# VITA-Group/mm-hand

Hardware: AMD Instinct MI355X
Metric: 256x256 hand images/sec (G+D step) (higher is better)
Workload: dtype f32; 1 GPU; RHD-shaped 256x256, per-GPU batch 32, fp32 (Winograd F(6x6,3x3) on the 3x3 stack), G(9 PATBlocks, ngf64)+D_PB+D_PP+L1/perceptual/GAN+Adam, --norm instance, dropout on; VGG19[:4] weights: random-init (seed 1234): NOT the reference's pretrained objective; global_batch=32, parallelism=dp1

## Files before the change

### include/mmhand_hip.h

```cpp
#ifndef MMHAND_HIP_H
#define MMHAND_HIP_H

#include <stddef.h>
#include <stdint.h>

#ifdef __cplusplus
extern "C" {
#endif
#pragma GCC visibility push(default)

typedef void* mmh_stream_t;

enum { MMH_PAD_ZERO = 0, MMH_PAD_REFLECT = 1 };
enum { MMH_ACT_NONE = 0, MMH_ACT_RELU = 1, MMH_ACT_TANH = 2 };
enum { MMH_F32 = 0, MMH_BF16 = 1, MMH_FP16 = 2 };

typedef struct mmh_conv_desc {
    int32_t B, H, W;
    int32_t Cin, Cout;
    int32_t kh, kw;
    int32_t stride;
    int32_t pad;
    int32_t pad_mode;
    int32_t Ho, Wo;
// ... 301 lines not shown
size_t mmh_conv7_head_dgrad_lp16_ws_bytes(const mmh_conv_desc* d);
int mmh_conv7_head_dgrad_lp16(const mmh_conv_desc* d, const void* dy, const void* w, void* dx, int dx_is16, void* ws,
                              size_t ws_bytes, const void* zeros, mmh_stream_t s);

int mmh_conv7_n4_lp16_supported(const mmh_conv_desc* d, int mode);
size_t mmh_conv7_n4_lp16_ws_bytes(const mmh_conv_desc* d, int mode);
int mmh_conv7_n4_lp16(const mmh_conv_desc* d, int mode, const void* x16, const void* w,
                      const void* bias, void* y, int act, void* ws, size_t ws_bytes,
                      const void* zeros, mmh_stream_t s);

int mmh_conv7_stem_wgrad_supported(const mmh_conv_desc* d);
size_t mmh_conv7_stem_wgrad_ws_bytes(const mmh_conv_desc* d);
int mmh_conv7_stem_wgrad(const mmh_conv_desc* d, const void* x, const void* dy, void* dw,
                         void* ws, size_t ws_bytes, int accumulate, mmh_stream_t s);

int mmh_adam_step(void* p, const void* g, void* m, void* v, int64_t n,
                  float lr, float beta1, float beta2, float eps, int step,
                  float grad_scale, const void* skip_flag, const void* loss_scale,
                  mmh_stream_t s);

int mmh_adam_step_dev(void* p, const void* g, void* m, void* v, int64_t n, const void* lr, float beta1, float beta2,
                      float eps, void* step, float grad_scale, const void* skip_flag, const void* loss_scale, void* coef,
                      mmh_stream_t s);

int mmh_set_dropout_salt(const void* salt_u64);
int mmh_u64_add(void* value_u64, uint64_t inc, mmh_stream_t s);

int mmh_pool_exchange(void* pool, const void* images, void* out, const void* src_idx, const void* dst_idx, int B,
                      int64_t elems_per_image, mmh_stream_t s);

// ... 110 lines not shown
```

### mmhand_amd/csrc/common.h

```cpp
#pragma once
#include <hip/hip_runtime.h>
#include <cstdarg>
#include <cstdio>
#include <cstdint>
#include "../../include/mmhand_hip.h"

namespace mmh {

char* err_buf();
int fail(const char* fmt, ...);

inline int check_launch(const char* what) {
    hipError_t e = hipGetLastError();
    if (e != hipSuccess) return fail("%s: %s", what, hipGetErrorString(e));
    return 0;
}

inline hipStream_t as_stream(mmh_stream_t s) { return reinterpret_cast<hipStream_t>(s); }

inline int64_t cdiv(int64_t a, int64_t b) { return (a + b - 1) / b; }

int wino6_weights(const float* w, float* U, int Cin, int Cout, int flip_transpose, hipStream_t st);
int wino6_weights_multi(const long long* table, int n, long long total_blocks, hipStream_t st);
int wino6_input(const float* x, float* V, int B, int H, int W, int C, int reflect, int xcd, hipStream_t st);
// ... 16 lines not shown
                       hipStream_t st);
bool dgrad_s2_halo_ok(const mmh_conv_desc* d, int dx_cs, int act);
int launch_dgrad_s2_halo(const mmh_conv_desc* d, const void* dy, const void* w, const void* bias, void* dx, int dx_cs,
                         int act, hipStream_t st);
extern int g_dgrad_s2_halo, g_dgrad_s2_dbg;
bool wgrad_s2_strip_ok(const mmh_conv_desc* d);
size_t wgrad_s2_strip_ws_bytes(const mmh_conv_desc* d);
int launch_wgrad_s2_strip(const mmh_conv_desc* d, const void* x, const void* dy, void* dw, void* ws, size_t ws_bytes,
                          int accumulate, hipStream_t st);
extern int g_wgrad_s2_strip;
bool stem_f32_ok(const mmh_conv_desc* d);
int stem_f32_stats_chunks(const mmh_conv_desc* d);
int launch_stem_f32(const mmh_conv_desc* d, const void* x, const void* w, const void* bias, void* y, int act, float* stats,
                    hipStream_t st);
extern int g_stem_f32, g_stem_f32_dbg, g_stem_f32_levels;
bool wino_wgrad_dma_ok(int64_t tiles, int Cin, int Cout, int nbatch);
size_t wino_wgrad_dma_ws_bytes(int64_t tiles, int Cin, int Cout, int nbatch);
int launch_wino_wgrad_dma(const float* V, const float* Yh, int64_t tiles, int Cin, int Cout, int nbatch, float* ws, float* dU,
                          hipStream_t st);
extern int g_wino_wgrad_dma;
int launch_slab_reduce(const float* slab, float* dw, int64_t n4_total, int splits, int accumulate, int64_t n4, hipStream_t st);
bool conv_s2f_ok(const mmh_conv_desc* d, int mode);
bool conv_s1f_ok(const mmh_conv_desc* d, int mode);
int conv_s2f_stats_chunks(const mmh_conv_desc* d);
int launch_conv_s2f(const mmh_conv_desc* d, const void* x16, const void* w16, const void* bias, void* y, int y_is16, int act,
                    const void* zeros, hipStream_t st, float* stats = nullptr, int mode = 0);
bool conv_s2d_ok(const mmh_conv_desc* d, int mode);
int launch_conv_s2d(const mmh_conv_desc* d, const void* g16, const void* w16, const void* bias, void* dx, int dx_is16, int act,
                    const void* zeros, hipStream_t st);
extern int g_lp16_s2f;
// ... 18 lines not shown
```

### mmhand_amd/csrc/conv_igemm.hip

```cpp
#include <algorithm>
#include <cstring>
#include "device_prims.h"

namespace {
using namespace mmh::dev;

typedef __bf16 bf16x4 __attribute__((ext_vector_type(4)));
typedef __bf16 bf16x2 __attribute__((ext_vector_type(2)));
typedef _Float16 f16x4 __attribute__((ext_vector_type(4)));
typedef _Float16 f16x2 __attribute__((ext_vector_type(2)));
__device__ __forceinline__ bf16x4 to_bf16x4(float4 v) {
    bf16x4 r;
    r[0] = (__bf16)v.x; r[1] = (__bf16)v.y; r[2] = (__bf16)v.z; r[3] = (__bf16)v.w;
    return r;
}
template <bool H16>
__device__ __forceinline__ bf16x4 to_lp4(float4 v) {
    if (H16) {
        f16x4 r;
        r[0] = (_Float16)v.x; r[1] = (_Float16)v.y; r[2] = (_Float16)v.z; r[3] = (_Float16)v.w;
        return __builtin_bit_cast(bf16x4, r);
    }
    return to_bf16x4(v);
}
// ... 2923 lines not shown
        {"wino_wgrad_dma", &mmh::g_wino_wgrad_dma},
        {"stem_f32_dbg", &mmh::g_stem_f32_dbg},
        {"slab_reduce_par", &mmh::g_slab_reduce_par},
        {"dgrad_s2_dbg", &mmh::g_dgrad_s2_dbg},
        {"lp16_dbg", &mmh::g_lp16_dbg},
        {"lp16_wgrad_ring", &mmh::g_lp16_wgrad_ring},
        {"lp16_wgrad_s2", &mmh::g_lp16_wgrad_s2},
        {"border_bn64", &g_border_bn64},
        {"wino_gemm_occ", &g_wino_gemm_occ},
        {"wino_gemm_levels", &g_wino_gemm_levels},
        {"wino_gemm_bn", &g_wino_gemm_bn},
        {"wino_bf16_occ", &g_wino_bf16_occ},
        {"wino_bf16_bk", &g_wino_bf16_bk},
        {"wino_wgrad_bn256", &g_wino_wgrad_bn256},
        {"wino_wgrad_slots", &g_wino_wgrad_slots},
    };
    *count = (int)(sizeof(table) / sizeof(table[0]));
    return table;
}
const OptionEntry* find_option(const char* key) {
    int n = 0;
    const OptionEntry* t = option_table(&n);
    for (int i = 0; i < n; ++i)
        if (!strcmp(key, t[i].name)) return &t[i];
    return nullptr;
}

}

extern "C" {
// ... 493 lines not shown
```

### mmhand_amd/lib.py

```python
import ctypes as C
import os

_HERE = os.path.dirname(os.path.abspath(__file__))
LIB_PATH = os.environ.get("MMH_LIB_PATH") or os.path.join(_HERE, "libmmhand_hip.so")

PAD_ZERO, PAD_REFLECT = 0, 1
ACT_NONE, ACT_RELU, ACT_TANH = 0, 1, 2
F32, BF16, FP16 = 0, 1, 2
U8 = 3


class ConvDesc(C.Structure):
    _fields_ = [(n, C.c_int32) for n in (
        "B", "H", "W", "Cin", "Cout", "kh", "kw", "stride", "pad", "pad_mode",
        "Ho", "Wo", "x_cs", "y_cs", "dtype")]


class PlaneSrc(C.Structure):
    _fields_ = [("ptr", C.c_void_p), ("C", C.c_int32),
                ("sb", C.c_int64), ("sc", C.c_int64), ("sh", C.c_int64), ("sw", C.c_int64)]


class ImageSrc(C.Structure):
    _fields_ = [("ptr", C.c_void_p), ("dtype", C.c_int32), ("scale", C.c_float), ("offset", C.c_float),
# ... 36 lines not shown
    "mmh_norm_stats_merge2": (_i, [_vp, _i, _i, _i, _vp, _sz, _vp, _vp, _vp]),
    "mmh_norm_stats_merge_finalize": (_i, [_vp, _i, _i, _i, _d, _f, _vp, _vp, _vp, _vp, _vp, _vp]),
    "mmh_wino_wgrad_gemm_ws_bytes": (_sz, [_i64, _i, _i, _i]),
    "mmh_wino_wgrad_gemm": (_i, [_vp, _vp, _i64, _i, _i, _i, _i, _vp, _sz, _vp, _vp]),
    "mmh_wino_dw": (_i, [_vp, _i, _i, _i, _vp, _i, _vp]),
    "mmh_conv2d_dgrad_border_ws_bytes": (_sz, [_DP]),
    "mmh_conv2d_dgrad_border": (_i, [_DP, _vp, _vp, _vp, _vp, _sz, _i, _i, _vp]),
    "mmh_conv7_thin_fprop": (_i, [_DP, _vp, _vp, _vp, _vp, _i, _vp]),
    "mmh_conv7_thin_dgrad_ws_bytes": (_sz, [_DP]),
    "mmh_conv7_thin_dgrad": (_i, [_DP, _vp, _vp, _vp, _vp, _sz, _i, _vp]),
    "mmh_conv7_thin_wgrad_ws_bytes": (_sz, [_DP]),
    "mmh_conv7_thin_wgrad": (_i, [_DP, _vp, _vp, _vp, _vp, _sz, _i, _vp]),
    "mmh_conv7_stem_wgrad_supported": (_i, [_DP]),
    "mmh_conv7_stem_wgrad_ws_bytes": (_sz, [_DP]),
    "mmh_conv7_stem_wgrad": (_i, [_DP, _vp, _vp, _vp, _vp, _sz, _i, _vp]),
    "mmh_conv2d_wgrad_ws_bytes": (_sz, [_DP]),
    "mmh_conv2d_wgrad": (_i, [_DP, _vp, _vp, _vp, _vp, _sz, _i, _i, _vp]),
    "mmh_convT2d_fprop": (_i, [_DP, _vp, _vp, _vp, _vp, _i, _i, _vp]),
    "mmh_convT2d_dgrad": (_i, [_DP, _vp, _vp, _vp, _vp]),
    "mmh_convT2d_wgrad": (_i, [_DP, _vp, _vp, _vp, _vp, _sz, _i, _i, _vp]),
    "mmh_reflect_fold": (_i, [_vp, _vp, _i, _i, _i, _i, _i, _vp]),
    "mmh_prep_weights_bf16": (_i, [_vp, _i, _i, _i, _vp, _vp, _vp]),
    "mmh_prep_weights_bf16_flat": (_i, [_vp, _i, _i, _i, _vp, _vp]),
    "mmh_prep_weights_fp16": (_i, [_vp, _i, _i, _i, _vp, _vp, _vp]),
    "mmh_prep_weights_fp16_flat": (_i, [_vp, _i, _i, _i, _vp, _vp]),
    "mmh_cvt_lp16": (_i, [_vp, _i64, _i, _vp, _vp]),
    "mmh_conv_lp16_supported": (_i, [_DP, _i]),
    "mmh_conv_lp16": (_i, [_DP, _i, _vp, _vp, _vp, _vp, _i, _i, _vp, _vp]),
    "mmh_conv_lp16_stats_chunks": (_i, [_DP]),
    "mmh_conv_lp16_fprop_stats": (_i, [_DP, _vp, _vp, _vp, _vp, _vp, _vp, _vp]),
# ... 163 lines not shown
```

### mmhand_amd/mmhand_model.py

```python
import os
import random
from collections import OrderedDict

import torch
import torch.distributed as dist

from . import lib as L
from . import ops
from .networks import Discriminator, Generator, VGGHead, discriminators_lockstep
from .ops import pad4
from .options import check_exact_fwd, check_resize_inputs


MERGE_D_PASSES = os.environ.get("MMH_MERGE_D", "1") != "0"
_LAST_BUCKET_LOG = None


def get_norm_layer(norm_type="instance"):
    if norm_type in ("batch", "instance"):
        return norm_type
    raise NotImplementedError("normalization layer [%s] is not found" % norm_type)


def get_scheduler(optimizer, opt):
# ... 257 lines not shown
        ops.set_dropout_seed((int(seed) * 0x9E3779B97F4A7C15 + 0x5EED0001 + rank * 0xD1B54A32D192ED03) % (1 << 64))
        norm = get_norm_layer(opt.norm)
        input_nc = [opt.H_input_nc, opt.P_input_nc * 2, opt.D_input_nc * 2]
        self.netG = Generator(input_nc, opt.output_nc, opt.ngf, norm, not opt.no_dropout,
                              n_blocks=getattr(opt, "G_n_blocks", 9),
                              n_downsampling=opt.G_n_downsampling)
        self.netG.to(self.device).init_weights(opt.init_type, seed)
        nets = [self.netG]
        if self.isTrain:
            self.netD_PB = Discriminator(opt.H_input_nc + opt.P_input_nc, opt.ndf, norm,
                                         not opt.no_dropout_D, opt.n_layers_D,
                                         n_downsampling=opt.D_n_downsampling)
            self.netD_PP = Discriminator(opt.H_input_nc + opt.H_input_nc, opt.ndf, norm,
                                         not opt.no_dropout_D, opt.n_layers_D,
                                         n_downsampling=opt.D_n_downsampling)
            self.netD_PB.to(self.device).init_weights(opt.init_type, seed + 1)
            self.netD_PP.to(self.device).init_weights(opt.init_type, seed + 2)
            nets += [self.netD_PB, self.netD_PP]
        if not self.isTrain or opt.continue_train:
            self.load_network()
        for n in nets:
            n.flatten_parameters()
        level = str(getattr(opt, "opt_level", "O0")).upper()
        if level not in ("O0", "O1", "O2", "O1_FP16", "O2_FP16", "BF16"):
            raise ValueError("--opt_level %r: expected O0 | O1 | O2 | O1_FP16 | O2_FP16 | BF16 (apex's O3 = "
                             "pure fp16 weights is 'not recommended' by the reference and not built)"
                             % (opt.opt_level,))
        self.bf16 = 2 if level.endswith("_FP16") else level in ("O1", "O2", "BF16")
        self.loss_scaling = self.isTrain and level != "O0" and level != "BF16"
        for n in nets:
# ... 592 lines not shown
```

### mmhand_amd/networks.py

```python
import functools
import math

import torch
import torch.nn as nn

from . import lib as L
from . import ops
from .ops import pad4


class ConvParam(nn.Module):

    def __init__(self, cin, cout, k, bias, transposed=False):
        super().__init__()
        self.cin, self.cout, self.k, self.transposed = cin, cout, k, transposed
        a, b = (pad4(cout), pad4(cin)) if transposed else (pad4(cin), pad4(cout))
        self.weight = nn.Parameter(torch.zeros(k, k, a, b))
        self.bias = nn.Parameter(torch.zeros(pad4(cout))) if bias else None

    def logical_weight(self):
        w = self.weight.detach()
        if self.transposed:
            return w.permute(3, 2, 0, 1)[: self.cin, : self.cout]
        return w.permute(3, 2, 0, 1)[: self.cout, : self.cin]

    def set_logical(self, weight=None, bias=None):
        with torch.no_grad():
            if weight is not None:
                self.weight.zero_()
                self.logical_weight().copy_(weight)
            if bias is not None and self.bias is not None:
                self.bias.zero_()
                self.bias[: self.cout].copy_(bias)
# ... 217 lines not shown
            elif isinstance(m, NormParam):
                with torch.no_grad():
                    m.weight.copy_(1.0 + torch.randn(m.weight.shape, generator=g) * 0.02)
                    m.bias.zero_()
        return self

    def conv(self, cp, x, stride=1, pad=0, reflect=False, act=L.ACT_NONE, dx_channels=0, y_lp=False, to_norm=False,
             g_defer=False, res_tok=None, x_twin=None):
        x16 = None
        if isinstance(x, tuple):
            x, x16 = x
        if isinstance(x16, ops.NormDefer):
            return ops.Conv2dFn.apply(x, cp.weight, cp.bias, stride, pad, reflect, act, self.bf16, dx_channels, None,
                                      False, bool(to_norm and self.norm == "instance" and self.training), x16, g_defer)
        nb = bool(to_norm and self.training and (self.norm == "instance" or cp.bias is None))
        if x16 is not None:
            res_tok = None
        if y_lp:
            p, y16 = ops.Conv2dFn.apply(x, cp.weight, cp.bias, stride, pad, reflect, act, self.bf16, dx_channels, x16, True, nb,
                                        None, False, res_tok, x_twin)
            return p, y16
        return ops.Conv2dFn.apply(x, cp.weight, cp.bias, stride, pad, reflect, act, self.bf16, dx_channels, x16, False, nb,
                                  None, g_defer, res_tok, x_twin)

    def _lp_edge(self, cp, stride=1, reflect=True):
        if not (self.bf16 and self.training and cp is not None and cp.k == 3):
            return 0
        ws = cp.weight.shape
        if cp.transposed:
            return self.bf16 if ops.convT_lp16_ok(ws[3], ws[2], self.bf16) else 0
# ... 156 lines not shown
    def __init__(self, input_nc, output_nc, ngf=64, norm_layer=nn.BatchNorm2d, use_dropout=False,
                 n_blocks=6, gpu_ids=[], padding_type="reflect", n_downsampling=2):
        assert type(input_nc) == list and len(input_nc) == 3, \
            "The AttModule take input_nc in format of list only!!"
        assert n_blocks >= 0
        if padding_type != "reflect":
            raise NotImplementedError("padding [%s] is not implemented" % padding_type)
        super().__init__(norm_layer, use_dropout)
        self.input_nc, self.output_nc, self.ngf = list(input_nc), output_nc, ngf
        self.n_blocks, self.n_down = n_blocks, n_downsampling
        self.gpu_ids = gpu_ids
        m = self.model = Bag()
        for s, nc in zip((1, 2, 3), input_nc):
            d = m.put(f"stream{s}_down", Bag())
            self._conv(d, 1, nc, ngf, 7)
            self._normp(d, 2, ngf)
            for i in range(n_downsampling):
                c = ngf * 2 ** i
                self._conv(d, 4 + 3 * i, c, 2 * c, 3)
                self._normp(d, 5 + 3 * i, 2 * c)
        dim = ngf * 2 ** n_downsampling
        att = m.put("att", Bag())
        i2 = 6 if use_dropout else 5
        for b in range(n_blocks):
            blk = att.put(b, Bag())
            for s in (1, 2, 3):
                cb = blk.put(f"conv_block_stream{s}", Bag())
                wide = (s != 1) and b > 0
                cin = 2 * dim if wide else dim
                self._conv(cb, 1, cin, cin, 3)
# ... 138 lines not shown
        self._normp(m, 2, ngf)
        for i in range(n_downsampling):
            c = ngf * 2 ** i
            self._conv(m, 4 + 3 * i, c, 2 * c, 3)
            self._normp(m, 5 + 3 * i, 2 * c)
        dim = ngf * 2 ** n_downsampling
        i2 = 6 if use_dropout else 5
        base = 4 + 3 * n_downsampling
        for b in range(n_blocks):
            cb = m.put(base + b, Bag()).put("conv_block", Bag())
            self._conv(cb, 1, dim, dim, 3)
            self._normp(cb, 2, dim)
            self._conv(cb, i2, dim, dim, 3)
            self._normp(cb, i2 + 1, dim)

    def forward_nhwc(self, x, dx_channels=0):
        m = self.model
        first = m[4] if self.n_down > 0 else None
        Bx, Hx, Wx, _ = x.shape
        y = self.normact(m, 2, self.conv(m[1], x, 1, 3, True, dx_channels=dx_channels, to_norm=True,
                                         y_lp=self._lp_out_stem(m[1], Bx, Hx, Wx, x.requires_grad, dx_channels)), True,
                         out_lp=self._lp_edge(first, 2, False))
        base = 4 + 3 * self.n_down
        twin = None
        for i in range(self.n_down):
            cp = m[4 + 3 * i]
            out_lp = self._lp_edge(m[4 + 3 * (i + 1)], 2, False) if i + 1 < self.n_down else 0
            wt = self._twin_for(m[base]["conv_block"][1]) if (i + 1 == self.n_down and self.n_blocks > 0) else 0
            y = self.normact(m, 5 + 3 * i, self.conv(cp, y, 2, 1, False, y_lp=self._lp_out(cp, 2, False), to_norm=True), True,
                             out_lp=out_lp, want_twin=wt)
# ... 123 lines not shown
```

### mmhand_amd/ops.py

```python
import ctypes as C
import os
import weakref

import torch

from . import lib as L


def _ptr(t):
    return None if t is None else C.c_void_p(t.data_ptr())


_raw_stream = getattr(torch._C, "_cuda_getCurrentRawStream", None)
_raw_device = getattr(torch._C, "_cuda_getDevice", None)


def _stream():
    if _raw_stream is not None and _raw_device is not None:
        return C.c_void_p(_raw_stream(_raw_device()))
    return C.c_void_p(torch.cuda.current_stream().cuda_stream)


def _chk(t, name="tensor"):
    if not (t.is_cuda and t.dtype == torch.float32 and t.is_contiguous()):
# ... 341 lines not shown
        _pending_stats.clear()
    _pending_stats[y.data_ptr()] = (stats, tuple(y.shape), weakref.ref(y), y._version)


def _take_stats(x, peek=False):
    pend = _pending_stats.get(x.data_ptr())
    if pend is None:
        return None
    y = pend[2]()
    if pend[1] != tuple(x.shape) or y is None or y._version != pend[3] or x._version != pend[3]:
        del _pending_stats[x.data_ptr()]
        return None
    if not peek:
        del _pending_stats[x.data_ptr()]
    return pend


def _wino_conv(x, U, bias, Cout, reflect, act, tile, time_it=False, keep_V=False, bf16=False, want_stats=False,
               fold=False, pro=None, levels=0, levels16=0):
    B, H, W_, Cin = x.shape
    P = (tile + 2) ** 2
    if fold:
        tiles = B * (-(-(H + 2) // 6)) * (-(-(W_ + 2) // 6))
    else:
        tiles = B * (-(-H // tile)) * (-(-W_ // tile))
    dt = _dt(bf16)
    wd = _wd(bf16)
    V = torch.empty((P, tiles, Cin), dtype=wd, device=x.device)
    M = torch.empty((P, tiles, Cout), dtype=wd, device=x.device)
    y = _empty((B, H, W_, Cout), x)
# ... 169 lines not shown
            e0, e1 = fprop_timer.bracket()
            e0.record()
        y = raw_conv_lp16_flat(d, x, w, bias, act, bf16)
        if timed:
            e1.record()
        return y
    if bf16:
        d.dtype = _dt(bf16)
        w = bf16_weights(w, bf16)[1]
    _count_desc("mfma", d)
    if (want_stats and FUSE_NORM_STATS and not bf16 and act == L.ACT_NONE and (d.Ho * d.Wo) % 128 == 0
            and not (fprop_timer is not None and fprop_timer.want(d))):
        chunks = L.load().mmh_conv2d_fprop_stats_chunks(C.byref(d))
        if chunks > 0:
            stats = _empty((B, chunks // B, 3, Cout), x)
            L.call("mmh_conv2d_fprop_stats", C.byref(d), _ptr(x), _ptr(w), _ptr(bias), _ptr(y), _ptr(stats), _stream())
            _park_stats(y, stats)
            return y
    if fprop_timer is not None and fprop_timer.want(d):
        e0, e1 = fprop_timer.bracket()
        e0.record()
        L.call("mmh_conv2d_fprop", C.byref(d), _ptr(x), _ptr(w), _ptr(bias), _ptr(y), act, _stream())
        e1.record()
        return y
    L.call("mmh_conv2d_fprop", C.byref(d), _ptr(x), _ptr(w), _ptr(bias), _ptr(y), act, _stream())
    return y


USE_CONV7_N4 = os.environ.get("MMH_CONV7_N4", "1") != "0"


# ... 186 lines not shown
        dw = out if out is not None else _empty((k, k, Cin, Cout), x)
        L.call("mmh_conv2d_wgrad", C.byref(d), _ptr(x), _ptr(dy), _ptr(dw), _ptr(ws), ws.numel() * 4, int(out is not None),
               (1 if x.dtype != torch.float32 else 0) | (2 if dy.dtype != torch.float32 else 0), _stream())
        _count_desc("mfma", d)
        return dw
    wt = _wino_tile(B, H, W_, Cin, Cout, k, stride, pad, bf16, "wgrad")
    if wt:
        return raw_conv_wgrad_wino(x, dy, reflect, wt, bf16=bf16, out=out)
    d = conv_desc(B, H, W_, Cin, Cout, k, stride, pad, reflect)
    if USE_THIN and k == 7 and stride == 1 and pad == 3 and Cout == 4 and Cin % 64 == 0:
        ws = _ws(L.load().mmh_conv7_thin_wgrad_ws_bytes(C.byref(d)), x)
        dw = out if out is not None else _empty((k, k, Cin, Cout), x)
        L.call("mmh_conv7_thin_wgrad", C.byref(d), _ptr(x), _ptr(dy), _ptr(dw), _ptr(ws), ws.numel() * 4,
               int(out is not None), _stream())
        _count_desc("valu", d)
        return dw
    if USE_STEM_WGRAD and not bf16 and L.load().mmh_conv7_stem_wgrad_supported(C.byref(d)):
        ws = _ws(L.load().mmh_conv7_stem_wgrad_ws_bytes(C.byref(d)), x)
        dw = out if out is not None else _empty((k, k, Cin, Cout), x)
        L.call("mmh_conv7_stem_wgrad", C.byref(d), _ptr(x), _ptr(dy), _ptr(dw), _ptr(ws), ws.numel() * 4,
               int(out is not None), _stream())
        _count_desc("mfma", d)
        return dw
    if bf16:
        d.dtype = _dt(bf16)
    assert (d.Ho, d.Wo) == (dy.shape[1], dy.shape[2])
    nbytes = L.load().mmh_conv2d_wgrad_ws_bytes(C.byref(d))
    ws = _ws(nbytes, x)
    dw = out if out is not None else _empty((k, k, Cin, Cout), x)
    L.call("mmh_conv2d_wgrad", C.byref(d), _ptr(x), _ptr(dy), _ptr(dw), _ptr(ws),
# ... 1768 lines not shown
def raw_pack(srcs, B, H, W_, Cd, device, out=None, twin=0, twin_out=None, only16=False, keep_twin=False):
    arr = (L.PlaneSrc * len(srcs))()
    for i, (t, nchw, nch) in enumerate(srcs):
        assert t.dtype == torch.float32 and t.is_cuda
        p = _plane(t, nchw)
        p.C = nch
        arr[i] = p
    c8 = (Cd + 7) // 8 * 8
    tiled = USE_PACK_TWIN and Cd <= 56
    if only16:
        assert twin and out is None and tiled, "a 16-bit-only pack needs the tiled kernel (Cd <= 56, MMH_PACK_TWIN)"
    elif out is None:
        out = torch.empty((B, H, W_, Cd), dtype=torch.float32, device=device)
    else:
        assert tuple(out.shape) == (B, H, W_, Cd) and out.is_contiguous() and out.dtype == torch.float32
    if not tiled:
        L.call("mmh_pack_nhwc", arr, len(srcs), _ptr(out), B, H, W_, Cd, 0, _stream())
        return out
    x16p = None
    if twin:
        x16p = twin_out if twin_out is not None else torch.empty((B, H, W_, c8), dtype=_wd(twin), device=device)
        assert x16p.is_contiguous() and x16p.dtype == _wd(twin) and tuple(x16p.shape) == (B, H, W_, c8)
    L.call("mmh_pack_nhwc_lp16", arr, len(srcs), _ptr(out), _ptr(x16p), B, H, W_, Cd, c8, _dt(twin) if twin else L.BF16,
           _stream())
    if only16:
        return x16p
    if twin and twin_out is None:
        pack_twin_put(out, x16p, keep=keep_twin)
    return out

# ... 268 lines not shown
```

Before: 121.8 images/s.

## Add activity-mask sparse 7x7 stem fprop and wgrad for pose-heatmap inputs

Adds a kernel that computes a per-tile bitmask of nonzero input channels for pose-heatmap inputs, which are mostly zero. New sparse 7x7 stem fprop and wgrad kernels then skip channel/tile pairs that are all zero. The mask is cached per input tensor, keyed on pointer, version and capture state, and is marked only for the pose-input stems (G stream 2 and D_PB). It exploits data sparsity exactly, so results stay correct, but it adds a mask pass and cache invalidation logic that could go stale.

New measurement: 128.8 images/s, median of 6. +5.7%, better.

```diff
diff --git a/include/mmhand_hip.h b/include/mmhand_hip.h
--- a/include/mmhand_hip.h
+++ b/include/mmhand_hip.h
@@ -339,6 +339,16 @@
 int mmh_conv7_stem_wgrad(const mmh_conv_desc* d, const void* x, const void* dy, void* dw,
                          void* ws, size_t ws_bytes, int accumulate, mmh_stream_t s);
 
+size_t mmh_stem_activity_bytes(int B, int H, int W);
+int mmh_stem_activity(const void* x, int B, int H, int W, int C, void* mask, mmh_stream_t s);
+int mmh_conv7_stem_sparse_fprop_supported(const mmh_conv_desc* d);
+int mmh_conv7_stem_sparse_fprop(const mmh_conv_desc* d, const void* x, const void* mask, const void* w, const void* bias,
+                                void* y, void* stats, mmh_stream_t s);
+int mmh_conv7_stem_sparse_wgrad_supported(const mmh_conv_desc* d);
+size_t mmh_conv7_stem_sparse_wgrad_ws_bytes(const mmh_conv_desc* d);
+int mmh_conv7_stem_sparse_wgrad(const mmh_conv_desc* d, const void* x, const void* mask, const void* dy, void* dw, void* ws,
+                                size_t ws_bytes, int accumulate, mmh_stream_t s);
+
 int mmh_adam_step(void* p, const void* g, void* m, void* v, int64_t n,
                   float lr, float beta1, float beta2, float eps, int step,
                   float grad_scale, const void* skip_flag, const void* loss_scale,
diff --git a/mmhand_amd/csrc/common.h b/mmhand_amd/csrc/common.h
--- a/mmhand_amd/csrc/common.h
+++ b/mmhand_amd/csrc/common.h
@@ -54,6 +54,7 @@
 int launch_stem_f32(const mmh_conv_desc* d, const void* x, const void* w, const void* bias, void* y, int act, float* stats,
                     hipStream_t st);
 extern int g_stem_f32, g_stem_f32_dbg, g_stem_f32_levels;
+extern int g_stem_sparse;
 bool wino_wgrad_dma_ok(int64_t tiles, int Cin, int Cout, int nbatch);
 size_t wino_wgrad_dma_ws_bytes(int64_t tiles, int Cin, int Cout, int nbatch);
 int launch_wino_wgrad_dma(const float* V, const float* Yh, int64_t tiles, int Cin, int Cout, int nbatch, float* ws, float* dU,
diff --git a/mmhand_amd/csrc/conv_igemm.hip b/mmhand_amd/csrc/conv_igemm.hip
--- a/mmhand_amd/csrc/conv_igemm.hip
+++ b/mmhand_amd/csrc/conv_igemm.hip
@@ -2961,6 +2961,7 @@
         {"wino_bf16_bk", &g_wino_bf16_bk},
         {"wino_wgrad_bn256", &g_wino_wgrad_bn256},
         {"wino_wgrad_slots", &g_wino_wgrad_slots},
+        {"stem_sparse", &mmh::g_stem_sparse},
     };
     *count = (int)(sizeof(table) / sizeof(table[0]));
     return table;
diff --git a/mmhand_amd/csrc/stem_f32_epilogue.h b/mmhand_amd/csrc/stem_f32_epilogue.h
--- /dev/null
+++ b/mmhand_amd/csrc/stem_f32_epilogue.h
@@ -0,0 +1,55 @@
+#pragma once
+#include "device_prims.h"
+
+namespace mmh { namespace dev {
+
+template <int MT>
+__device__ __forceinline__ void stem_f32_epilogue(const f32x16* acc, float* y, float* stats, int tile, int b, int ty, int tx,
+                                                  int pg, int kg, int n, float bv, int H, int W, int y_cs, int act) {
+    constexpr int TR = 8 * MT, TC = 16;
+#pragma unroll
+    for (int mt = 0; mt < MT; ++mt) {
+#pragma unroll
+        for (int i = 0; i < 16; ++i) {
+            const int mm = (i & 3) + 8 * (i >> 2) + 4 * kg;
+            const int oh = ty * TR + 8 * mt + 2 * pg + (mm >> 4), ow = tx * TC + (mm & 15);
+            if (oh < H && ow < W)
+                y[((size_t)(b * H + oh) * W + ow) * (size_t)y_cs + n] = act_apply(acc[mt][i] + bv, act);
+        }
+    }
+    if (stats) {
+        float mean_w = 0.f, m2_w = 0.f;
+#pragma unroll
+        for (int mt = 0; mt < MT; ++mt) {
+            float sum = 0.f;
+#pragma unroll
+            for (int i = 0; i < 16; ++i) sum += acc[mt][i] + bv;
+            const float mean_l = sum * (1.f / 16.f);
+            float m2 = 0.f;
+#pragma unroll
+            for (int i = 0; i < 16; ++i) {
+                const float dv = acc[mt][i] + bv - mean_l;
+                m2 += dv * dv;
+            }
+            const float mean_o = __shfl_xor(mean_l, 32, 64), m2_o = __shfl_xor(m2, 32, 64);
+            const float dm = mean_o - mean_l;
+            const float mean_t = mean_l + 0.5f * dm, m2_t = m2 + m2_o + dm * dm * 8.f;
+            if (mt == 0) {
+                mean_w = mean_t;
+                m2_w = m2_t;
+            } else {
+                const float d2 = mean_t - mean_w;
+                mean_w += 0.5f * d2;
+                m2_w += m2_t + d2 * d2 * 16.f;
+            }
+        }
+        if (kg == 0) {
+            float* o = stats + ((size_t)(tile * 4 + pg) * 3) * 64 + n;
+            o[0] = 32.f * MT;
+            o[64] = mean_w;
+            o[128] = m2_w;
+        }
+    }
+}
+
+} }
diff --git a/mmhand_amd/csrc/stem_sparse.hip b/mmhand_amd/csrc/stem_sparse.hip
--- /dev/null
+++ b/mmhand_amd/csrc/stem_sparse.hip
@@ -0,0 +1,399 @@
+#include <algorithm>
+#include "stem_f32_epilogue.h"
+
+namespace mmh { int g_stem_sparse = 1; }
+
+namespace {
+using namespace mmh::dev;
+
+constexpr int BR = 8, BC = 16;
+constexpr int HC = BC + 6;
+constexpr int CMAX = 48;
+
+__device__ __forceinline__ int reflect_idx(int i, int n) {
+    i = i < 0 ? -i : i;
+    return i >= n ? 2 * (n - 1) - i : i;
+}
+
+__global__ void __launch_bounds__(256) stem_activity_kernel(const float* __restrict__ x, unsigned long long* __restrict__ mask,
+                                                            int H, int W, int C) {
+    __shared__ unsigned long long part[4];
+    const int bx = blockIdx.x, by = blockIdx.y, b = blockIdx.z;
+    const int c4 = C >> 2;
+    const int units = (BR + 6) * HC * c4;
+    unsigned long long bits = 0;
+    for (int u = threadIdx.x; u < units; u += 256) {
+        const int px = u / c4, q = u - px * c4;
+        const int hr = px / HC, hc = px - hr * HC;
+        const int ih = reflect_idx(by * BR - 3 + hr, H), iw = reflect_idx(bx * BC - 3 + hc, W);
+        const float4 v = *reinterpret_cast<const float4*>(x + ((size_t)(b * H + ih) * W + iw) * (size_t)C + 4 * q);
+        const unsigned nz = (v.x != 0.f ? 1u : 0u) | (v.y != 0.f ? 2u : 0u) | (v.z != 0.f ? 4u : 0u) | (v.w != 0.f ? 8u : 0u);
+        bits |= (unsigned long long)nz << (4 * q);
+    }
+#pragma unroll
+    for (int s = 32; s >= 1; s >>= 1) {
+        const unsigned lo = __shfl_xor((unsigned)bits, s, 64), hi = __shfl_xor((unsigned)(bits >> 32), s, 64);
+        bits |= ((unsigned long long)hi << 32) | lo;
+    }
+    if ((threadIdx.x & 63) == 0) part[threadIdx.x >> 6] = bits;
+    __syncthreads();
+    if (threadIdx.x == 0)
+        mask[((size_t)b * gridDim.y + by) * gridDim.x + bx] = part[0] | part[1] | part[2] | part[3];
+}
+
+constexpr int FNT = 512;
+constexpr int CAP_LO = 12, CH_LO = 98, CH_HI = 224;
+
+struct SparseFpropKP {
+    const float* x;
+    const unsigned long long* mask;
+    const float* w;
+    const float* bias;
+    float* y;
+    float* stats;
+    int B, H, W, Cin, x_cs, y_cs, J, TX, TY;
+    int cap, ch;
+    int lo, hi;
+};
+
+template <int MT>
+__global__ void __launch_bounds__(FNT, 1) stem_sparse_fprop_kernel(const SparseFpropKP p) {
+    constexpr int TR = 8 * MT, HR = TR + 6, PLANE = HR * HC;
+    extern __shared__ __attribute__((aligned(16))) char smem[];
+    const int tid = threadIdx.x;
+    const int lane = tid & 63, wave = tid >> 6;
+    const int m = lane & 31, kg = lane >> 5;
+    const int pg = wave & 3, nh = wave >> 2;
+    int* wave_cnt = reinterpret_cast<int*>(smem);
+    int2* ent = reinterpret_cast<int2*>(smem + 32);
+    const int ent_b = 32 + (((7 * p.Cin + 1) * 8 + 15) & ~15);
+    float* planes = reinterpret_cast<float*>(smem + ent_b);
+    float* wst = planes + (p.cap + 1) * PLANE;
+
+    const int tile = blockIdx.x;
+    const int tpi = p.TX * p.TY;
+    const int b = tile / tpi;
+    const int trem = tile - b * tpi;
+    const int ty = trem / p.TX, tx = trem - ty * p.TX;
+
+    unsigned long long act = 0;
+#pragma unroll
+    for (int mt = 0; mt < MT; ++mt) act |= p.mask[((size_t)b * (p.H / BR) + ty * MT + mt) * (p.W / BC) + tx];
+    const int nact = __popcll(act);
+    if (nact < p.lo || nact > p.hi) return;
+    const int Lr = 7 * nact, Lp = (Lr + 1) & ~1;
+    const int CH = p.ch;
+
+    {
+        const int g = tid >> 3, r = tid & 7;
+        const int j = 8 * g + 4 * (r & 1) + (r >> 1);
+        const int kw = j / p.Cin, c = j - kw * p.Cin;
+        const bool on = j < p.J && ((act >> c) & 1ull);
+        const unsigned long long bal = __ballot(on);
+        if (lane == 0) wave_cnt[wave] = __popcll(bal);
+        __syncthreads();
+        int rank = __popcll(bal & ((1ull << lane) - 1ull));
+        for (int v = 0; v < wave; ++v) rank += wave_cnt[v];
+        if (on) ent[rank] = make_int2(__popcll(act & ((1ull << c) - 1ull)) * (PLANE * 4) + 4 * kw, j);
+        if (tid == 0 && Lp > Lr) ent[Lr] = make_int2(nact * (PLANE * 4), 0);
+    }
+    for (int u = tid; u < (nact + 1) * PLANE; u += FNT) {
+        const int a = u / PLANE, px = u - a * PLANE;
+        float v = 0.f;
+        if (a < nact) {
+            unsigned long long t = act;
+            for (int i = 0; i < a; ++i) t &= t - 1;
+            const int c = __ffsll((long long)t) - 1;
+            const int hr = px / HC, hc = px - hr * HC;
+            const int ih = reflect_idx(ty * TR - 3 + hr, p.H), iw = reflect_idx(tx * BC - 3 + hc, p.W);
+            v = p.x[((size_t)(b * p.H + ih) * p.W + iw) * (size_t)p.x_cs + c];
+        }
+        planes[u] = v;
+    }
+
+    f32x16 acc[MT];
+#pragma unroll
+    for (int mt = 0; mt < MT; ++mt)
+#pragma unroll
+        for (int i = 0; i < 16; ++i) acc[mt][i] = 0.f;
+
+    const int a_lane = ((2 * pg + (m >> 4)) * HC + (m & 15)) * 4;
+    const int n = 32 * nh + m;
+    const char* const planes_c = reinterpret_cast<const char*>(planes);
+
+    const int khg = Lp <= CH ? (Lp ? min(7, CH / Lp) : 7) : 1;
+    const int cw = Lp <= CH ? Lp : CH;
+    for (int kh0 = 0; kh0 < 7; kh0 += khg) {
+        const int nk = min(khg, 7 - kh0);
+        for (int c0 = 0; c0 < Lp; c0 += cw) {
+            const int ne = min(cw, Lp - c0);
+            __syncthreads();
+            for (int u = tid; u < nk * ne * 16; u += FNT) {
+                const int rr = u >> 4, q = u & 15;
+                const int k = rr / ne, idx = rr - k * ne;
+                const int j = ent[c0 + idx].y;
+                *reinterpret_cast<float4*>(wst + rr * 64 + 4 * q) =
+                    *reinterpret_cast<const float4*>(p.w + ((size_t)(kh0 + k) * p.J + j) * 64 + 4 * q);
+            }
+            __syncthreads();
+            for (int k = 0; k < nk; ++k) {
+                const int arow = a_lane + (kh0 + k) * (HC * 4);
+                const float* wk = wst + k * ne * 64 + n;
+                for (int i = 0; i < ne; i += 2) {
+                    const int e = ent[c0 + i + kg].x;
+                    const float bw = wk[(i + kg) * 64];
+#pragma unroll
+                    for (int mt = 0; mt < MT; ++mt) {
+                        const float av = *reinterpret_cast<const float*>(planes_c + e + arow + mt * 8 * (HC * 4));
+                        acc[mt] = __builtin_amdgcn_mfma_f32_32x32x2f32(av, bw, acc[mt], 0, 0, 0);
+                    }
+                }
+            }
+        }
+    }
+    const float bv = p.bias ? p.bias[n] : 0.f;
+    stem_f32_epilogue<MT>(acc, p.y, p.stats, tile, b, ty, tx, pg, kg, n, bv, p.H, p.W, p.y_cs, MMH_ACT_NONE);
+}
+
+int dense_mt(const mmh_conv_desc* d) {
+    if (d->H % BR || d->W % BC) return 0;
+    const int chunks = mmh::stem_f32_stats_chunks(d);
+    if (chunks <= 0) return 0;
+    const int mt = d->B * (d->H / BR) * (d->W / BC) * 4 / chunks;
+    return (mt == 1 || mt == 2) ? mt : 0;
+}
+
+size_t fprop_lds(int Cin, int mt, int cap, int ch) {
+    return 32 + (size_t)(((7 * Cin + 1) * 8 + 15) & ~15) + (size_t)(cap + 1) * (8 * mt + 6) * HC * 4 + (size_t)ch * 256;
+}
+
+bool fprop_ok(const mmh_conv_desc* d) {
+    if (!d || !mmh::stem_f32_ok(d) || d->pad_mode != MMH_PAD_REFLECT || d->Cin > CMAX) return false;
+    if (mmh::g_stem_f32_levels != 1) return false;
+    const int mt = dense_mt(d);
+    return mt && d->H >= 4 && d->W >= 4 && fprop_lds(d->Cin, mt, d->Cin, CH_HI) <= 160 * 1024;
+}
+
+constexpr int WNT = 256;
+constexpr int WTR = 2, WTC = 64;
+constexpr int WP = WTR * WTC;
+constexpr int WHC = WTC + 6, WHPL = (WTR + 6) * WHC;
+constexpr int WNH = (WHPL + WNT - 1) / WNT;
+
+struct SparseWgradKP {
+    const float* x;
+    const unsigned long long* mask;
+    const float* dy;
+    float* slab;
+    int H, W, Cin, x_cs, y_cs, BX, BY, tw, th, tiles, tiles_per_split;
+};
+
+__device__ __forceinline__ void wgrad_fetch(const SparseWgradKP& p, int t, int c, int tid, float4 (&dreg)[8], float (&hreg)[WNH]) {
+    const int wx = t % p.tw, hy = (t / p.tw) % p.th, b = t / (p.tw * p.th);
+#pragma unroll
+    for (int u = 0; u < 8; ++u) {
+        const int e = u * WNT + tid;
+        const int px = e >> 4, q = e & 15;
+        const int oh = hy * WTR + (px >> 6), ow = wx * WTC + (px & 63);
+        dreg[u] = *reinterpret_cast<const float4*>(p.dy + ((size_t)(b * p.H + oh) * p.W + ow) * (size_t)p.y_cs + 4 * q);
+    }
+#pragma unroll
+    for (int u = 0; u < WNH; ++u) {
+        const int e = min(u * WNT + tid, WHPL - 1);
+        const int hr = e / WHC, hc = e - hr * WHC;
+        const int ih = reflect_idx(hy * WTR - 3 + hr, p.H), iw = reflect_idx(wx * WTC - 3 + hc, p.W);
+        hreg[u] = p.x[((size_t)(b * p.H + ih) * p.W + iw) * (size_t)p.x_cs + c];
+    }
+}
+
+__global__ void __launch_bounds__(WNT) stem_sparse_wgrad_kernel(const SparseWgradKP p) {
+    extern __shared__ __attribute__((aligned(16))) char smem[];
+    __shared__ int wave_cnt[4];
+    float* dys = reinterpret_cast<float*>(smem);
+    float* halo = dys + WP * 64;
+    int* list = reinterpret_cast<int*>(halo + WHPL);
+    const int tid = threadIdx.x, lane = tid & 63, wave = tid >> 6;
+    const int m = lane & 31, kg = lane >> 5;
+    const int mh = wave & 1, nh = wave >> 1;
+    const int c = blockIdx.x, split = blockIdx.y;
+    const int t0 = split * p.tiles_per_split;
+    const int nt = max(0, min(p.tiles_per_split, p.tiles - t0));
+
+    int nlist = 0;
+    for (int i0 = 0; i0 < nt; i0 += WNT) {
+        const int i = i0 + tid;
+        bool on = false;
+        if (i < nt) {
+            const int t = t0 + i;
+            const int wx = t % p.tw, hy = (t / p.tw) % p.th, b = t / (p.tw * p.th);
+            const unsigned long long* mw = p.mask + ((size_t)b * p.BY + (hy * WTR) / BR) * p.BX + wx * (WTC / BC);
+            on = (((mw[0] | mw[1] | mw[2] | mw[3]) >> c) & 1ull) != 0;
+        }
+        const unsigned long long bal = __ballot(on);
+        if (lane == 0) wave_cnt[wave] = __popcll(bal);
+        __syncthreads();
+        int rank = nlist + __popcll(bal & ((1ull << lane) - 1ull));
+        for (int v = 0; v < wave; ++v) rank += wave_cnt[v];
+        if (on) list[rank] = t0 + i;
+        nlist += wave_cnt[0] + wave_cnt[1] + wave_cnt[2] + wave_cnt[3];
+        __syncthreads();
+    }
+
+    f32x16 acc;
+#pragma unroll
+    for (int i = 0; i < 16; ++i) acc[i] = 0.f;
+    const int tap = min(32 * mh + m, 48);
+    const int a_lane = (tap / 7) * WHC + (tap % 7);
+
+    float4 dreg[8];
+    float hreg[WNH];
+#pragma unroll
+    for (int u = 0; u < 8; ++u) dreg[u] = make_float4(0.f, 0.f, 0.f, 0.f);
+#pragma unroll
+    for (int u = 0; u < WNH; ++u) hreg[u] = 0.f;
+    if (nlist > 0) wgrad_fetch(p, list[0], c, tid, dreg, hreg);
+    for (int a = 0; a < nlist; ++a) {
+#pragma unroll
+        for (int u = 0; u < 8; ++u) *reinterpret_cast<float4*>(dys + (u * WNT + tid) * 4) = dreg[u];
+#pragma unroll
+        for (int u = 0; u < WNH; ++u)
+            if (u * WNT + tid < WHPL) halo[u * WNT + tid] = hreg[u];
+        __syncthreads();
+        if (a + 1 < nlist) wgrad_fetch(p, list[a + 1], c, tid, dreg, hreg);
+        const float* bcol = dys + 32 * nh + m;
+#pragma unroll 8
+        for (int i = 0; i < WP / 2; ++i) {
+            const int px = 2 * i + kg;
+            const float av = halo[a_lane + (px >> 6) * WHC + (px & 63)];
+            const float bw = bcol[px * 64];
+            acc = __builtin_amdgcn_mfma_f32_32x32x2f32(av, bw, acc, 0, 0, 0);
+        }
+        __syncthreads();
+    }
+    float* out = p.slab + (size_t)split * 49 * p.Cin * 64 + (size_t)c * 64 + 32 * nh + m;
+#pragma unroll
+    for (int r = 0; r < 16; ++r) {
+        const int t = 32 * mh + (r & 3) + 8 * (r >> 2) + 4 * kg;
+        if (t < 49) out[(size_t)t * p.Cin * 64] = acc[r];
+    }
+}
+
+bool wgrad_ok(const mmh_conv_desc* d) {
+    return d && d->kh == 7 && d->kw == 7 && d->stride == 1 && d->pad == 3 && d->pad_mode == MMH_PAD_REFLECT &&
+           d->dtype == MMH_F32 && d->Cout == 64 && d->y_cs >= 64 && d->y_cs % 4 == 0 && d->Cin >= 4 && d->Cin <= CMAX &&
+           d->Cin % 4 == 0 && d->x_cs >= d->Cin && d->H % BR == 0 && d->W % WTC == 0 && d->H >= 4 && d->W >= 4 &&
+           d->Ho == d->H && d->Wo == d->W && d->B >= 1 &&
+           (size_t)d->B * d->H * d->W * std::max(d->x_cs, d->y_cs) < (1ull << 31);
+}
+
+void wgrad_splits(const mmh_conv_desc* d, int& tiles, int& tiles_per_split, int& splits) {
+    tiles = d->B * (d->H / WTR) * (d->W / WTC);
+    int khg = (14 * 32) / (7 * d->Cin);
+    khg = khg < 1 ? 1 : (khg > 7 ? 7 : khg);
+    const int groups = (7 + khg - 1) / khg;
+    splits = std::max(1, 512 / groups);
+    splits = std::min(splits, tiles);
+    tiles_per_split = (tiles + splits - 1) / splits;
+}
+
+bool mask_args_ok(int B, int H, int W) {
+    return B >= 1 && H >= 4 && W >= 4 && H % BR == 0 && W % BC == 0;
+}
+
+}
+
+extern "C" {
+
+size_t mmh_stem_activity_bytes(int B, int H, int W) {
+    return mask_args_ok(B, H, W) ? (size_t)B * (H / BR) * (W / BC) * 8 : 0;
+}
+
+int mmh_stem_activity(const void* x, int B, int H, int W, int C, void* mask, mmh_stream_t s) {
+    MMH_REQUIRE(mask_args_ok(B, H, W), "mmh_stem_activity: needs H %% 8 == 0, W %% 16 == 0, H, W >= 4 (got %d x %d x %d)", B, H, W);
+    MMH_REQUIRE(C >= 4 && C <= CMAX && C % 4 == 0, "mmh_stem_activity: needs 4 <= C <= 48, C %% 4 == 0 (got %d)", C);
+    MMH_REQUIRE((size_t)B * H * W * C < (1ull << 31), "mmh_stem_activity: tensor too large");
+    MMH_REQUIRE(x && mask, "mmh_stem_activity: NULL buffer");
+    MMH_REQUIRE(((uintptr_t)x & 15) == 0 && ((uintptr_t)mask & 7) == 0, "mmh_stem_activity: x needs 16-byte, mask 8-byte alignment");
+    MMH_REQUIRE(H / BR <= 65535 && B <= 65535, "mmh_stem_activity: grid too large");
+    hipLaunchKernelGGL(stem_activity_kernel, dim3(W / BC, H / BR, B), dim3(256), 0, mmh::as_stream(s),
+                       static_cast<const float*>(x), static_cast<unsigned long long*>(mask), H, W, C);
+    return mmh::check_launch("stem_activity_kernel");
+}
+
+int mmh_conv7_stem_sparse_fprop_supported(const mmh_conv_desc* d) { return mmh::g_stem_sparse && fprop_ok(d) ? 1 : 0; }
+
+int mmh_conv7_stem_sparse_fprop(const mmh_conv_desc* d, const void* x, const void* mask, const void* w, const void* bias,
+                                void* y, void* stats, mmh_stream_t s) {
+    MMH_REQUIRE(fprop_ok(d), "mmh_conv7_stem_sparse_fprop: needs an fp32 7x7 / stride 1 / reflect pad 3 stem, Cin %% 4 == 0 "
+                             "<= 48, Cout == 64, whole dense-kernel tiles, conv_levels 1");
+    MMH_REQUIRE(x && mask && w && y, "mmh_conv7_stem_sparse_fprop: NULL buffer");
+    MMH_REQUIRE(((uintptr_t)w & 15) == 0 && ((uintptr_t)mask & 7) == 0 && ((uintptr_t)x & 3) == 0 && ((uintptr_t)y & 3) == 0,
+                "mmh_conv7_stem_sparse_fprop: w needs 16-byte, mask 8-byte alignment");
+    const int mt = dense_mt(d);
+    SparseFpropKP p{};
+    p.x = static_cast<const float*>(x);
+    p.mask = static_cast<const unsigned long long*>(mask);
+    p.w = static_cast<const float*>(w);
+    p.bias = static_cast<const float*>(bias);
+    p.y = static_cast<float*>(y);
+    p.stats = static_cast<float*>(stats);
+    p.B = d->B; p.H = d->H; p.W = d->W; p.Cin = d->Cin; p.x_cs = d->x_cs; p.y_cs = d->y_cs; p.J = 7 * d->Cin;
+    p.TX = d->W / BC; p.TY = d->H / (BR * mt);
+    static int ready = -1;
+    if (ready != 0) {
+        for (const void* k : {reinterpret_cast<const void*>(stem_sparse_fprop_kernel<1>), reinterpret_cast<const void*>(stem_sparse_fprop_kernel<2>)}) {
+            hipError_t e = hipFuncSetAttribute(k, hipFuncAttributeMaxDynamicSharedMemorySize, 160 * 1024);
+            if (e != hipSuccess) return mmh::fail("mmh_conv7_stem_sparse_fprop: %s", hipGetErrorString(e));
+        }
+        ready = 0;
+    }
+    const int tiles = p.B * p.TX * p.TY;
+    for (int pass = 0; pass < 2; ++pass) {
+        if (pass == 0) { p.cap = std::min(CAP_LO, d->Cin); p.ch = CH_LO; p.lo = 0; p.hi = p.cap; }
+        else { p.cap = d->Cin; p.ch = CH_HI; p.lo = CAP_LO + 1; p.hi = d->Cin; }
+        if (p.lo > p.hi) break;
+        const size_t lds = fprop_lds(d->Cin, mt, p.cap, p.ch);
+        if (mt == 2) hipLaunchKernelGGL(stem_sparse_fprop_kernel<2>, dim3(tiles), dim3(FNT), lds, mmh::as_stream(s), p);
+        else hipLaunchKernelGGL(stem_sparse_fprop_kernel<1>, dim3(tiles), dim3(FNT), lds, mmh::as_stream(s), p);
+        if (int rc = mmh::check_launch("stem_sparse_fprop_kernel")) return rc;
+    }
+    return 0;
+}
+
+int mmh_conv7_stem_sparse_wgrad_supported(const mmh_conv_desc* d) { return mmh::g_stem_sparse && wgrad_ok(d) ? 1 : 0; }
+
+size_t mmh_conv7_stem_sparse_wgrad_ws_bytes(const mmh_conv_desc* d) {
+    if (!wgrad_ok(d)) return 0;
+    int tiles, per, splits;
+    wgrad_splits(d, tiles, per, splits);
+    return (size_t)splits * 49 * d->Cin * 64 * sizeof(float);
+}
+
+int mmh_conv7_stem_sparse_wgrad(const mmh_conv_desc* d, const void* x, const void* mask, const void* dy, void* dw, void* ws,
+                                size_t ws_bytes, int accumulate, mmh_stream_t s) {
+    MMH_REQUIRE(wgrad_ok(d), "mmh_conv7_stem_sparse_wgrad: needs an fp32 7x7 / stride 1 / reflect pad 3 stem, Cin %% 4 == 0 <= 48, "
+                             "Cout == 64, H %% 8 == 0, W %% 64 == 0");
+    MMH_REQUIRE(x && mask && dy && dw && ws && ws_bytes >= mmh_conv7_stem_sparse_wgrad_ws_bytes(d),
+                "mmh_conv7_stem_sparse_wgrad: bad buffers");
+    MMH_REQUIRE(((uintptr_t)dy & 15) == 0 && ((uintptr_t)dw & 15) == 0 && ((uintptr_t)ws & 15) == 0 && ((uintptr_t)mask & 7) == 0 &&
+                    ((uintptr_t)x & 3) == 0,
+                "mmh_conv7_stem_sparse_wgrad: dy, dw, ws need 16-byte, mask 8-byte alignment");
+    SparseWgradKP p{};
+    p.x = static_cast<const float*>(x);
+    p.mask = static_cast<const unsigned long long*>(mask);
+    p.dy = static_cast<const float*>(dy);
+    p.slab = static_cast<float*>(ws);
+    p.H = d->H; p.W = d->W; p.Cin = d->Cin; p.x_cs = d->x_cs; p.y_cs = d->y_cs;
+    p.BX = d->W / BC; p.BY = d->H / BR; p.tw = d->W / WTC; p.th = d->H / WTR;
+    int splits;
+    wgrad_splits(d, p.tiles, p.tiles_per_split, splits);
+    const size_t lds = (size_t)(WP * 64 + WHPL + p.tiles_per_split) * sizeof(float);
+    MMH_REQUIRE(lds <= 64 * 1024, "mmh_conv7_stem_sparse_wgrad: tile list does not fit LDS");
+    hipStream_t st = mmh::as_stream(s);
+    hipLaunchKernelGGL(stem_sparse_wgrad_kernel, dim3(d->Cin, splits), dim3(WNT), lds, st, p);
+    if (int rc = mmh::check_launch("stem_sparse_wgrad_kernel")) return rc;
+    const int n4 = 49 * d->Cin * 64 / 4;
+    return mmh::launch_slab_reduce(p.slab, static_cast<float*>(dw), n4, splits, accumulate, n4, st);
+}
+
+}
diff --git a/mmhand_amd/lib.py b/mmhand_amd/lib.py
--- a/mmhand_amd/lib.py
+++ b/mmhand_amd/lib.py
@@ -74,6 +74,13 @@
     "mmh_conv7_stem_wgrad_supported": (_i, [_DP]),
     "mmh_conv7_stem_wgrad_ws_bytes": (_sz, [_DP]),
     "mmh_conv7_stem_wgrad": (_i, [_DP, _vp, _vp, _vp, _vp, _sz, _i, _vp]),
+    "mmh_stem_activity_bytes": (_sz, [_i, _i, _i]),
+    "mmh_stem_activity": (_i, [_vp, _i, _i, _i, _i, _vp, _vp]),
+    "mmh_conv7_stem_sparse_fprop_supported": (_i, [_DP]),
+    "mmh_conv7_stem_sparse_fprop": (_i, [_DP, _vp, _vp, _vp, _vp, _vp, _vp, _vp]),
+    "mmh_conv7_stem_sparse_wgrad_supported": (_i, [_DP]),
+    "mmh_conv7_stem_sparse_wgrad_ws_bytes": (_sz, [_DP]),
+    "mmh_conv7_stem_sparse_wgrad": (_i, [_DP, _vp, _vp, _vp, _vp, _vp, _sz, _i, _vp]),
     "mmh_conv2d_wgrad_ws_bytes": (_sz, [_DP]),
     "mmh_conv2d_wgrad": (_i, [_DP, _vp, _vp, _vp, _vp, _sz, _i, _i, _vp]),
     "mmh_convT2d_fprop": (_i, [_DP, _vp, _vp, _vp, _vp, _i, _i, _vp]),
diff --git a/mmhand_amd/mmhand_model.py b/mmhand_amd/mmhand_model.py
--- a/mmhand_amd/mmhand_model.py
+++ b/mmhand_amd/mmhand_model.py
@@ -295,6 +295,7 @@
             self.netD_PP = Discriminator(opt.H_input_nc + opt.H_input_nc, opt.ndf, norm,
                                          not opt.no_dropout_D, opt.n_layers_D,
                                          n_downsampling=opt.D_n_downsampling)
+            self.netD_PB.stem_conv().pose_input = True
             self.netD_PB.to(self.device).init_weights(opt.init_type, seed + 1)
             self.netD_PP.to(self.device).init_weights(opt.init_type, seed + 2)
             nets += [self.netD_PB, self.netD_PP]
diff --git a/mmhand_amd/networks.py b/mmhand_amd/networks.py
--- a/mmhand_amd/networks.py
+++ b/mmhand_amd/networks.py
@@ -17,6 +17,7 @@
         a, b = (pad4(cout), pad4(cin)) if transposed else (pad4(cin), pad4(cout))
         self.weight = nn.Parameter(torch.zeros(k, k, a, b))
         self.bias = nn.Parameter(torch.zeros(pad4(cout))) if bias else None
+        self.pose_input = False
 
     def logical_weight(self):
         w = self.weight.detach()
@@ -264,6 +265,8 @@
             return ops.Conv2dFn.apply(x, cp.weight, cp.bias, stride, pad, reflect, act, self.bf16, dx_channels, None,
                                       False, bool(to_norm and self.norm == "instance" and self.training), x16, g_defer)
         nb = bool(to_norm and self.training and (self.norm == "instance" or cp.bias is None))
+        if cp.pose_input and nb and x16 is None and not self.bf16 and cp.k == 7 and stride == 1 and pad == 3 and reflect:
+            ops.stem_mask_request(x, cp.weight.shape[3])
         if x16 is not None:
             res_tok = None
         if y_lp:
@@ -450,6 +453,7 @@
         for s, nc in zip((1, 2, 3), input_nc):
             d = m.put(f"stream{s}_down", Bag())
             self._conv(d, 1, nc, ngf, 7)
+            d[1].pose_input = s == 2
             self._normp(d, 2, ngf)
             for i in range(n_downsampling):
                 c = ngf * 2 ** i
@@ -618,6 +622,9 @@
             self._conv(cb, i2, dim, dim, 3)
             self._normp(cb, i2 + 1, dim)
 
+    def stem_conv(self):
+        return self.model[1]
+
     def forward_nhwc(self, x, dx_channels=0):
         m = self.model
         first = m[4] if self.n_down > 0 else None
diff --git a/mmhand_amd/ops.py b/mmhand_amd/ops.py
--- a/mmhand_amd/ops.py
+++ b/mmhand_amd/ops.py
@@ -379,6 +379,47 @@
     if not peek:
         del _pending_stats[x.data_ptr()]
     return pend
+
+
+_stem_masks = {}
+
+
+def _stem_mask_for(x):
+    ent = _stem_masks.get(x.data_ptr())
+    if ent is None:
+        return None
+    if (ent[1] != tuple(x.shape) or ent[2] != x._version or ent[3]() is None
+            or ent[4] != torch.cuda.is_current_stream_capturing()):
+        return None
+    return ent[0]
+
+
+def stem_mask_forget(t):
+    _stem_masks.pop(t.data_ptr(), None)
+
+
+def stem_mask_request(x, cout=64):
+    if not (torch.is_tensor(x) and x.is_cuda and x.dtype == torch.float32 and x.dim() == 4 and x.is_contiguous()):
+        return None
+    B, H, W_, Cc = x.shape
+    nbytes = L.load().mmh_stem_activity_bytes(B, H, W_)
+    if nbytes == 0 or Cc % 4 or not 4 <= Cc <= 48 or x.numel() >= 2 ** 31 or x.data_ptr() % 16:
+        return None
+    d = conv_desc(B, H, W_, Cc, cout, 7, 1, 3, True)
+    if not (L.load().mmh_conv7_stem_sparse_fprop_supported(C.byref(d))
+            or (USE_STEM_WGRAD and L.load().mmh_conv7_stem_wgrad_supported(C.byref(d))
+                and L.load().mmh_conv7_stem_sparse_wgrad_supported(C.byref(d)))):
+        return None
+    mask = _stem_mask_for(x)
+    if mask is not None:
+        return mask
+    if len(_stem_masks) >= 8:
+        for k in [k for k, e in _stem_masks.items() if e[3]() is None]:
+            del _stem_masks[k]
+    mask = torch.empty((nbytes // 8,), dtype=torch.int64, device=x.device)
+    L.call("mmh_stem_activity", _ptr(x), B, H, W_, Cc, _ptr(mask), _stream())
+    _stem_masks[x.data_ptr()] = (mask, tuple(x.shape), x._version, weakref.ref(x), torch.cuda.is_current_stream_capturing())
+    return mask
 
 
 def _wino_conv(x, U, bias, Cout, reflect, act, tile, time_it=False, keep_V=False, bf16=False, want_stats=False,
@@ -578,7 +619,12 @@
         chunks = L.load().mmh_conv2d_fprop_stats_chunks(C.byref(d))
         if chunks > 0:
             stats = _empty((B, chunks // B, 3, Cout), x)
-            L.call("mmh_conv2d_fprop_stats", C.byref(d), _ptr(x), _ptr(w), _ptr(bias), _ptr(y), _ptr(stats), _stream())
+            mask = _stem_mask_for(x)
+            if mask is not None and L.load().mmh_conv7_stem_sparse_fprop_supported(C.byref(d)):
+                L.call("mmh_conv7_stem_sparse_fprop", C.byref(d), _ptr(x), _ptr(mask), _ptr(w), _ptr(bias), _ptr(y),
+                       _ptr(stats), _stream())
+            else:
+                L.call("mmh_conv2d_fprop_stats", C.byref(d), _ptr(x), _ptr(w), _ptr(bias), _ptr(y), _ptr(stats), _stream())
             _park_stats(y, stats)
             return y
     if fprop_timer is not None and fprop_timer.want(d):
@@ -795,6 +841,15 @@
         L.call("mmh_conv7_thin_wgrad", C.byref(d), _ptr(x), _ptr(dy), _ptr(dw), _ptr(ws), ws.numel() * 4,
                int(out is not None), _stream())
         _count_desc("valu", d)
+        return dw
+    mask = None if (bf16 or not x.is_contiguous()) else _stem_mask_for(x)
+    if (mask is not None and dy.is_contiguous() and USE_STEM_WGRAD and L.load().mmh_conv7_stem_wgrad_supported(C.byref(d))
+            and L.load().mmh_conv7_stem_sparse_wgrad_supported(C.byref(d))):
+        ws = _ws(L.load().mmh_conv7_stem_sparse_wgrad_ws_bytes(C.byref(d)), x)
+        dw = out if out is not None else _empty((k, k, Cin, Cout), x)
+        L.call("mmh_conv7_stem_sparse_wgrad", C.byref(d), _ptr(x), _ptr(mask), _ptr(dy), _ptr(dw), _ptr(ws), ws.numel() * 4,
+               int(out is not None), _stream())
+        _count_desc("mfma", d)
         return dw
     if USE_STEM_WGRAD and not bf16 and L.load().mmh_conv7_stem_wgrad_supported(C.byref(d)):
         ws = _ws(L.load().mmh_conv7_stem_wgrad_ws_bytes(C.byref(d)), x)
@@ -2593,6 +2648,7 @@
         out = torch.empty((B, H, W_, Cd), dtype=torch.float32, device=device)
     else:
         assert tuple(out.shape) == (B, H, W_, Cd) and out.is_contiguous() and out.dtype == torch.float32
+        stem_mask_forget(out)
     if not tiled:
         L.call("mmh_pack_nhwc", arr, len(srcs), _ptr(out), B, H, W_, Cd, 0, _stream())
         return out
```
